# renegade-fi/mpc-jellyfish

Hardware: AMD Instinct MI355X
Metric: msm_g1_scalar_pairs_per_s (higher is better)
Workload: dtype u32 (381-bit Fq as 14 x 29-bit limbs, Montgomery)

## Files before the change

### mpc-jellyfish_amd/csrc/ecz.cuh

```cuda
#pragma once
#include "ecx.cuh"
#include "fz.cuh"

namespace mzk {

template <class Z>
struct AffineZ {
    Fz<Z> x, y;
    MZK_HD bool is_inf() const {
        int32_t a = 0;
#pragma unroll
        for (int i = 0; i < Z::ZN; i++) a |= x.l[i] | y.l[i];
        return a == 0;
    }
};

template <class Z>
struct XYZZZ {
    Fz<Z> x, y, zz, zzz;
    MZK_HD bool is_inf() const { return fz_is_zero(zz); }
    MZK_HD static XYZZZ inf() {
        XYZZZ r;
        r.x = Fz<Z>::one(); r.y = Fz<Z>::one(); r.zz = Fz<Z>::zero(); r.zzz = Fz<Z>::zero();
        return r;
    }
    MZK_HD static XYZZZ from_affine(const AffineZ<Z>& p) {
        if (p.is_inf()) return inf();
        XYZZZ r;
        r.x = p.x; r.y = p.y; r.zz = Fz<Z>::one(); r.zzz = Fz<Z>::one();
        return r;
    }
};

template <class Z>
MZK_HD void ecz_xy3(Fz<Z>& x3, Fz<Z>& y3, const Fz<Z>& a, const Fz<Z>& b_plus_2c, const Fz<Z>& q, const Fz<Z>& r, const Fz<Z>& y, const Fz<Z>& ppp) {
    x3 = fz_norm_wide(fz_sub(a, b_plus_2c));
    const Fz<Z> d = fz_norm(fz_sub(q, x3));
    y3 = fz_mul2(r, d, y, fz_neg(ppp));
}

template <class Z>
MZK_HD XYZZZ<Z> xyzzz_dbl_affine(const AffineZ<Z>& p) {
    XYZZZ<Z> r;
    const Fz<Z> u = fz_norm(fz_add(p.y, p.y));
    const Fz<Z> v = fz_sqr(u);
    const Fz<Z> w = fz_mul(u, v);
    const Fz<Z> s = fz_mul(p.x, v);
    const Fz<Z> x2 = fz_sqr(p.x);
    const Fz<Z> m = fz_norm_wide(fz_add(fz_add(x2, x2), x2));
    const Fz<Z> mm = fz_sqr(m);
    ecz_xy3<Z>(r.x, r.y, mm, fz_add(s, s), s, m, p.y, w);
    r.zz = v;
    r.zzz = w;
    return r;
}

template <class Z>
MZK_HD XYZZZ<Z> xyzzz_dbl(const XYZZZ<Z>& p) {
    if (p.is_inf()) return p;
    XYZZZ<Z> r;
    const Fz<Z> u = fz_norm(fz_add(p.y, p.y));
    const Fz<Z> v = fz_sqr(u);
    const Fz<Z> w = fz_mul(u, v);
    const Fz<Z> s = fz_mul(p.x, v);
    const Fz<Z> x2 = fz_sqr(p.x);
    const Fz<Z> m = fz_norm_wide(fz_add(fz_add(x2, x2), x2));
    const Fz<Z> mm = fz_sqr(m);
    ecz_xy3<Z>(r.x, r.y, mm, fz_add(s, s), s, m, p.y, w);
    r.zz = fz_mul(v, p.zz);
    r.zzz = fz_mul(w, p.zzz);
    return r;
}

template <class Z>
MZK_HD XYZZZ<Z> xyzzz_madd(const XYZZZ<Z>& p, const AffineZ<Z>& q, bool negate) {
    if (q.is_inf()) return p;
    const Fz<Z> qy = negate ? fz_neg(q.y) : q.y;
    if (p.is_inf()) {
        XYZZZ<Z> r;
        r.x = q.x; r.y = qy; r.zz = Fz<Z>::one(); r.zzz = Fz<Z>::one();
        return r;
    }
    const Fz<Z> u2 = fz_mul(q.x, p.zz);
    const Fz<Z> s2 = fz_mul(qy, p.zzz);
    const Fz<Z> pp_ = fz_norm(fz_sub(u2, p.x));
    const Fz<Z> rr_ = fz_norm(fz_sub(s2, p.y));
    const Fz<Z> pp = fz_sqr(pp_);
    const Fz<Z> rr2 = fz_sqr(rr_);
    if (fz_is_zero(pp)) {
        if (fz_is_zero(rr2)) {
            AffineZ<Z> qq;
            qq.x = q.x;
            qq.y = qy;
            return xyzzz_dbl_affine(qq);
        }
        return XYZZZ<Z>::inf();
    }
    XYZZZ<Z> r;
    const Fz<Z> ppp = fz_mul(pp_, pp);
    const Fz<Z> qv = fz_mul(p.x, pp);
    ecz_xy3<Z>(r.x, r.y, rr2, fz_add(ppp, fz_add(qv, qv)), qv, rr_, p.y, ppp);
    r.zz = fz_mul(p.zz, pp);
    r.zzz = fz_mul(p.zzz, ppp);
    return r;
}

template <class Z>
MZK_HD XYZZZ<Z> xyzzz_add(const XYZZZ<Z>& p, const XYZZZ<Z>& q) {
    if (q.is_inf()) return p;
    if (p.is_inf()) return q;
    const Fz<Z> u1 = fz_mul(p.x, q.zz), u2 = fz_mul(q.x, p.zz);
    const Fz<Z> s1 = fz_mul(p.y, q.zzz), s2 = fz_mul(q.y, p.zzz);
    const Fz<Z> pp_ = fz_norm(fz_sub(u2, u1));
    const Fz<Z> rr_ = fz_norm(fz_sub(s2, s1));
    const Fz<Z> pp = fz_sqr(pp_);
    const Fz<Z> rr2 = fz_sqr(rr_);
    if (fz_is_zero(pp)) {
        if (fz_is_zero(rr2)) return xyzzz_dbl(p);
        return XYZZZ<Z>::inf();
    }
    XYZZZ<Z> r;
    const Fz<Z> ppp = fz_mul(pp_, pp);
    const Fz<Z> qv = fz_mul(u1, pp);
    ecz_xy3<Z>(r.x, r.y, rr2, fz_add(ppp, fz_add(qv, qv)), qv, rr_, s1, ppp);
    r.zz = fz_mul(fz_mul(p.zz, q.zz), pp);
    r.zzz = fz_mul(fz_mul(p.zzz, q.zzz), ppp);
    return r;
}

#if defined(__HIPCC__)
template <int CTRL, class Z>
__device__ __forceinline__ Fz<Z> fz_quad_perm(const Fz<Z>& a) {
    Fz<Z> r;
#pragma unroll
    for (int i = 0; i < Z::ZN; i++) {
        r.l[i] = __builtin_amdgcn_update_dpp(0, a.l[i], CTRL, 0xF, 0xF, true);
        asm("" : "+v"(r.l[i]));
    }
    return r;
}
template <class Z>
__device__ __forceinline__ Fz<Z> fz_sel(bool c, const Fz<Z>& a, const Fz<Z>& b) {
    Fz<Z> r;
#pragma unroll
    for (int i = 0; i < Z::ZN; i++) r.l[i] = c ? a.l[i] : b.l[i];
    return r;
}

template <class Z>
__device__ __forceinline__ Fz<Z> xyzzz_add_quad(const Fz<Z>& ca, const Fz<Z>& cb, int role) {
    const bool r0 = role == 0, r1 = role == 1, hi = role >= 2;
    int special = (role == 2 && (fz_is_zero(ca) || fz_is_zero(cb))) ? 1 : 0;
    const Fz<Z> p1 = fz_mul(ca, fz_quad_perm<QP_SWAP2>(cb));
    const Fz<Z> d = fz_norm(fz_sub(fz_quad_perm<QP_SWAP2>(p1), p1));
    const Fz<Z> p2 = fz_mul(fz_sel(hi, ca, d), fz_sel(hi, cb, d));
    if (r0 && fz_is_zero(p2)) special = 1;
    special |= __builtin_amdgcn_update_dpp(0, special, QP_SWAP1, 0xF, 0xF, true);
    special |= __builtin_amdgcn_update_dpp(0, special, QP_SWAP2, 0xF, 0xF, true);
    if (special) {
        XYZZZ<Z> a, b;
        a.x = fz_quad_perm<QP_L0>(ca); a.y = fz_quad_perm<QP_L1>(ca); a.zz = fz_quad_perm<QP_L2>(ca); a.zzz = fz_quad_perm<QP_L3>(ca);
        b.x = fz_quad_perm<QP_L0>(cb); b.y = fz_quad_perm<QP_L1>(cb); b.zz = fz_quad_perm<QP_L2>(cb); b.zzz = fz_quad_perm<QP_L3>(cb);
        const XYZZZ<Z> r = xyzzz_add(a, b);
        return fz_sel(hi, fz_sel(role == 2, r.zz, r.zzz), fz_sel(r0, r.x, r.y));
    }
    const Fz<Z> pp = fz_quad_perm<QP_L0>(p2);
    const Fz<Z> u1 = fz_quad_perm<QP_L0>(p1);
    const Fz<Z> p3 = fz_mul(fz_sel(r0, d, fz_sel(r1, u1, p2)), pp);
    const Fz<Z> ppp = fz_quad_perm<QP_L0>(p3);
    const Fz<Z> x3 = fz_norm_wide(fz_sub(p2, fz_add(ppp, fz_add(p3, p3))));
    const Fz<Z> qx = fz_norm(fz_sub(p3, x3));
    const Fz<Z> s1 = fz_quad_perm<QP_L1>(p1);
    const Fz<Z> p4 = fz_mul(fz_sel(r0, s1, fz_sel(r1, d, p2)), fz_sel(r1, qx, ppp));
    const Fz<Z> y3 = fz_norm(fz_sub(p4, fz_quad_perm<QP_L0>(p4)));
    const Fz<Z> x3_0 = fz_quad_perm<QP_L1>(x3);
    return fz_sel(hi, fz_sel(role == 2, p3, p4), fz_sel(r0, x3_0, y3));
}
#endif

// ... 11 lines not shown
```

### mpc-jellyfish_amd/csrc/fz.cuh

```cuda
#pragma once
#include "fp.cuh"

namespace mzk {

template <class Z>
struct Fz {
    static constexpr int N = Z::ZN;
    int32_t l[N];
    MZK_HD static Fz zero() {
        Fz r;
#pragma unroll
        for (int i = 0; i < N; i++) r.l[i] = 0;
        return r;
    }
    MZK_HD static Fz from_const(const int32_t (&c)[Z::ZN]) {
        Fz r;
#pragma unroll
        for (int i = 0; i < N; i++) r.l[i] = c[i];
        return r;
    }
    MZK_HD static Fz one() { return from_const(Z::ZONE); }
};

MZK_HD int32_t fz_sext(uint32_t v) { return (int32_t)(v << 2) >> 2; }
template <class Z>
MZK_HD int32_t fz_p_limb(int i) {
    int32_t v = Z::ZP[i];
#if defined(__HIP_DEVICE_COMPILE__)
    asm("" : "+s"(v));
#endif
    return v;
}

template <class Z>
MZK_HD Fz<Z> fz_mul(const Fz<Z>& x, const Fz<Z>& y) {
    constexpr int N = Z::ZN;
    int32_t m[N], pl[N];
#pragma unroll
    for (int i = 0; i < N; i++) pl[i] = fz_p_limb<Z>(i);
    Fz<Z> t;
    int64_t acc = 0;
#pragma unroll
    for (int k = 0; k < N; k++) {
#pragma unroll
        for (int i = 0; i <= k; i++) acc += (int64_t)x.l[i] * y.l[k - i];
#pragma unroll
        for (int i = 0; i < k; i++) acc += (int64_t)m[i] * pl[k - i];
        m[k] = fz_sext((uint32_t)acc * Z::ZINV);
        acc += (int64_t)m[k] * pl[0];
        acc >>= Z::ZL;
    }
#pragma unroll
    for (int k = N; k < 2 * N - 1; k++) {
#pragma unroll
        for (int i = k - N + 1; i < N; i++) {
            acc += (int64_t)x.l[i] * y.l[k - i];
            acc += (int64_t)m[i] * pl[k - i];
        }
        t.l[k - N] = fz_sext((uint32_t)acc);
        acc = (acc + (1 << (Z::ZL - 1))) >> Z::ZL;
    }
    t.l[N - 1] = (int32_t)acc;
    return t;
}
template <class Z>
MZK_HD Fz<Z> fz_mul2(const Fz<Z>& x, const Fz<Z>& y, const Fz<Z>& u, const Fz<Z>& v) {
    constexpr int N = Z::ZN;
    int32_t m[N], pl[N];
#pragma unroll
    for (int i = 0; i < N; i++) pl[i] = fz_p_limb<Z>(i);
    Fz<Z> t;
    int64_t acc = 0;
#pragma unroll
    for (int k = 0; k < N; k++) {
#pragma unroll
        for (int i = 0; i <= k; i++) {
            acc += (int64_t)x.l[i] * y.l[k - i];
            acc += (int64_t)u.l[i] * v.l[k - i];
        }
#pragma unroll
        for (int i = 0; i < k; i++) acc += (int64_t)m[i] * pl[k - i];
        m[k] = fz_sext((uint32_t)acc * Z::ZINV);
        acc += (int64_t)m[k] * pl[0];
        acc >>= Z::ZL;
    }
#pragma unroll
    for (int k = N; k < 2 * N - 1; k++) {
#pragma unroll
        for (int i = k - N + 1; i < N; i++) {
            acc += (int64_t)x.l[i] * y.l[k - i];
            acc += (int64_t)u.l[i] * v.l[k - i];
            acc += (int64_t)m[i] * pl[k - i];
        }
        t.l[k - N] = fz_sext((uint32_t)acc);
        acc = (acc + (1 << (Z::ZL - 1))) >> Z::ZL;
    }
    t.l[N - 1] = (int32_t)acc;
    return t;
}
template <class Z>
MZK_HD Fz<Z> fz_sqr(const Fz<Z>& x) {
    constexpr int N = Z::ZN;
    int32_t m[N], pl[N], x2[N];
#pragma unroll
    for (int i = 0; i < N; i++) { pl[i] = fz_p_limb<Z>(i); x2[i] = x.l[i] * 2; }
    Fz<Z> t;
    int64_t acc = 0;
#pragma unroll
    for (int k = 0; k < N; k++) {
#pragma unroll
        for (int i = 0; 2 * i < k; i++) acc += (int64_t)x.l[i] * x2[k - i];
        if (k % 2 == 0) acc += (int64_t)x.l[k / 2] * x.l[k / 2];
#pragma unroll
        for (int i = 0; i < k; i++) acc += (int64_t)m[i] * pl[k - i];
        m[k] = fz_sext((uint32_t)acc * Z::ZINV);
        acc += (int64_t)m[k] * pl[0];
        acc >>= Z::ZL;
    }
#pragma unroll
    for (int k = N; k < 2 * N - 1; k++) {
#pragma unroll
        for (int i = k - N + 1; 2 * i < k; i++) acc += (int64_t)x.l[i] * x2[k - i];
        if (k % 2 == 0) acc += (int64_t)x.l[k / 2] * x.l[k / 2];
#pragma unroll
        for (int i = k - N + 1; i < N; i++) acc += (int64_t)m[i] * pl[k - i];
        t.l[k - N] = fz_sext((uint32_t)acc);
        acc = (acc + (1 << (Z::ZL - 1))) >> Z::ZL;
    }
    t.l[N - 1] = (int32_t)acc;
    return t;
}

template <class Z>
MZK_HD Fz<Z> fz_add(const Fz<Z>& a, const Fz<Z>& b) {
    Fz<Z> r;
#pragma unroll
    for (int i = 0; i < Z::ZN; i++) r.l[i] = a.l[i] + b.l[i];
    return r;
}
template <class Z>
MZK_HD Fz<Z> fz_sub(const Fz<Z>& a, const Fz<Z>& b) {
    Fz<Z> r;
#pragma unroll
    for (int i = 0; i < Z::ZN; i++) r.l[i] = a.l[i] - b.l[i];
    return r;
}
template <class Z>
MZK_HD Fz<Z> fz_neg(const Fz<Z>& a) {
    Fz<Z> r;
#pragma unroll
    for (int i = 0; i < Z::ZN; i++) r.l[i] = -a.l[i];
    return r;
}

template <class Z>
MZK_HD Fz<Z> fz_norm(const Fz<Z>& a) {
    constexpr int N = Z::ZN, L = Z::ZL;
    Fz<Z> r;
    r.l[0] = fz_sext((uint32_t)a.l[0]);
#pragma unroll
    for (int i = 1; i < N - 1; i++) r.l[i] = fz_sext((uint32_t)a.l[i]) + ((a.l[i - 1] + (1 << (L - 1))) >> L);
    r.l[N - 1] = a.l[N - 1] + ((a.l[N - 2] + (1 << (L - 1))) >> L);
    return r;
}
template <class Z>
MZK_HD Fz<Z> fz_norm_wide(const Fz<Z>& a) {
    constexpr int N = Z::ZN, L = Z::ZL;
    Fz<Z> r;
    r.l[0] = fz_sext((uint32_t)a.l[0]);
#pragma unroll
    for (int i = 1; i < N - 1; i++) r.l[i] = fz_sext((uint32_t)a.l[i]) + (((a.l[i - 1] >> (L - 1)) + 1) >> 1);
    r.l[N - 1] = a.l[N - 1] + (((a.l[N - 2] >> (L - 1)) + 1) >> 1);
    return r;
}
template <class Z>
MZK_HD Fz<Z> fz_carry(const Fz<Z>& a) {
    constexpr int N = Z::ZN, L = Z::ZL;
    Fz<Z> r;
    int32_t c = 0;
#pragma unroll
    for (int i = 0; i < N - 1; i++) {
        const int32_t t = a.l[i] + c;
        r.l[i] = fz_sext((uint32_t)t);
        c = ((t >> (L - 1)) + 1) >> 1;
    }
    r.l[N - 1] = a.l[N - 1] + c;
    return r;
}
template <class Z>
MZK_HD bool fz_is_zero(const Fz<Z>& a) {
    int32_t z = 0;
#pragma unroll
    for (int i = 0; i < Z::ZN; i++) z |= a.l[i];
    return z == 0;
}
template <class Z>
MZK_HD Fz<Z> fz_canonical(const Fz<Z>& a) {
    constexpr int N = Z::ZN, L = Z::ZL;
    constexpr int32_t MASK = (1 << L) - 1;
    Fz<Z> r;
    int32_t c = 0;
#pragma unroll
    for (int i = 0; i < N - 1; i++) {
        const int32_t t = a.l[i] + c;
        r.l[i] = t & MASK;
        c = t >> L;
    }
    r.l[N - 1] = a.l[N - 1] + c;
// ... 79 lines not shown
```

### mpc-jellyfish_amd/csrc/msm.cuh

```cuda
#pragma once
#include <hip/hip_runtime.h>

#include "ec.cuh"
#include "ecx.cuh"
#include "ecz.cuh"

namespace mzk {

constexpr int MSM_THREADS = 256;
constexpr int MSM_ACC_THREADS = 128;
constexpr uint32_t MSM_HEAVY_PER_THREAD = 16;
constexpr uint32_t MSM_HEAVY_RUN = MSM_ACC_THREADS * MSM_HEAVY_PER_THREAD;
constexpr uint32_t MSM_HEAVY_FANIN = MSM_ACC_THREADS * 32;
constexpr int MSM_HEAVY_COUNTERS = 6;
__host__ __device__ inline bool msm_is_heavy(uint32_t count, uint32_t cap) { return count > cap + MSM_HEAVY_RUN; }

inline int msm_choose_window(unsigned long long n) {
    int lg = 0;
    while ((1ull << (lg + 1)) <= n) lg++;
    int c = lg - 2;
    if (c < 4) c = 4;
    if (c > 16) c = 16;
    return c;
}
// ... 152 lines not shown
        order[(size_t)row * M + pos] = w * M + b;
    }
}

struct LongDesc;
struct HeavyRun;
__device__ __forceinline__ void msm_long_register(uint32_t w, uint32_t b, uint32_t c, uint32_t offs_t, int n_win, uint32_t cap, uint32_t desc_cap,
                                                  LongDesc* __restrict__ desc, uint32_t* __restrict__ desc_count, uint32_t run_cap,
                                                  uint32_t h1_cap, HeavyRun* __restrict__ heavy_runs);
__global__ __launch_bounds__(1024) void msm_order_place_kernel(const uint32_t* __restrict__ hist, const uint32_t* __restrict__ offs, uint32_t M,
                                                               const uint32_t* __restrict__ keycnt, uint32_t* __restrict__ keycur, uint32_t* __restrict__ order,
                                                               int n_win, uint32_t cap, uint32_t desc_cap, LongDesc* __restrict__ desc,
                                                               uint32_t* __restrict__ desc_count, uint32_t run_cap, uint32_t h1_cap, HeavyRun* __restrict__ heavy_runs,
                                                               bool global) {
    __shared__ uint32_t cnt[1024];
    __shared__ uint32_t part[1024];
    const uint32_t w = blockIdx.y, t = threadIdx.x;
    const uint32_t row = global ? 0u : w;
    const uint32_t lo = blockIdx.x * MSM_ORDER_SLICE, hi = min(M, lo + MSM_ORDER_SLICE);
    uint32_t total = 0;
    if (global) for (uint32_t s = 0; s < gridDim.y; s++) total += keycnt[(size_t)s * 1024 + t];
    else total = keycnt[(size_t)w * 1024 + t];
    part[t] = total;
    cnt[t] = 0;
    __syncthreads();
    for (int d = 1; d < 1024; d <<= 1) {
        uint32_t v = t >= (uint32_t)d ? part[t - d] : 0;
        __syncthreads();
        part[t] += v;
        __syncthreads();
    }
    const uint32_t key_start = part[t] - total;
    for (uint32_t b = lo + t; b < hi; b += 1024) atomicAdd(&cnt[order_key(hist[(size_t)w * M + b])], 1u);
    __syncthreads();
    const uint32_t mine = cnt[t];
    __syncthreads();
    cnt[t] = mine ? key_start + atomicAdd(&keycur[(size_t)row * 1024 + t], mine) : 0u;
    __syncthreads();
    for (uint32_t b = lo + t; b < hi; b += 1024) {
        const uint32_t c = hist[(size_t)w * M + b];
        const uint32_t pos = atomicAdd(&cnt[order_key(c)], 1u);
        order[(size_t)row * M + pos] = w * M + b;
        if (desc_count && c > cap) msm_long_register(w, b, c, offs[(size_t)w * M + b], n_win, cap, desc_cap, desc, desc_count, run_cap, h1_cap, heavy_runs);
    }
}

template <class FQ>
__device__ __forceinline__ Affine<Fp<FQ>> load_affine(const uint32_t* __restrict__ bases, unsigned long long idx) {
    Affine<Fp<FQ>> p;
    const uint32_t* src = bases + idx * (2 * FQ::N);
    p.x = load_fp<FQ>(src);
    p.y = load_fp<FQ>(src + FQ::N);
    return p;
}
template <class FQ>
__device__ __forceinline__ XYZZ<Fp<FQ>> load_xyzz(const uint32_t* __restrict__ buf, unsigned long long idx) {
    XYZZ<Fp<FQ>> p;
    const uint32_t* src = buf + idx * (4 * FQ::N);
    p.x = load_fp<FQ>(src);
    p.y = load_fp<FQ>(src + FQ::N);
    p.zz = load_fp<FQ>(src + 2 * FQ::N);
    p.zzz = load_fp<FQ>(src + 3 * FQ::N);
    return p;
}
template <class FQ>
__device__ __forceinline__ void store_xyzz(uint32_t* __restrict__ buf, unsigned long long idx, const XYZZ<Fp<FQ>>& p) {
    uint32_t* dst = buf + idx * (4 * FQ::N);
    store_fp<FQ>(dst, p.x);
    store_fp<FQ>(dst + FQ::N, p.y);
    store_fp<FQ>(dst + 2 * FQ::N, p.zz);
    store_fp<FQ>(dst + 3 * FQ::N, p.zzz);
}

template <class FQ>
struct EcFp {
    using Field = FQ;
    using Aff = Affine<Fp<FQ>>;
    using Pt = XYZZ<Fp<FQ>>;
    static constexpr int AFF_WORDS = 2 * FQ::N, PT_WORDS = 4 * FQ::N;
    static __device__ __forceinline__ Aff load_aff(const uint32_t* __restrict__ bases, unsigned long long idx) { return load_affine<FQ>(bases, idx); }
    static __device__ __forceinline__ Pt load_pt(const uint32_t* __restrict__ buf, unsigned long long idx) { return load_xyzz<FQ>(buf, idx); }
    static __device__ __forceinline__ void store_pt(uint32_t* __restrict__ buf, unsigned long long idx, const Pt& p) { store_xyzz<FQ>(buf, idx, p); }
    static __device__ __forceinline__ Pt inf() { return Pt::inf(); }
    static __device__ __forceinline__ Pt madd(const Pt& a, Aff q, bool negate) {
        if (negate) q.y = neg(q.y);
        return xyzz_madd(a, q);
    }
    static __device__ __forceinline__ Pt add(const Pt& a, const Pt& b) { return xyzz_add(a, b); }
    static __device__ __forceinline__ XYZZ<Fp<FQ>> to_boundary(const Pt& p) { return p; }
};

template <class X>
__device__ __forceinline__ void load_words(uint32_t* dst, const uint32_t* __restrict__ src, int n_words) {
    for (int i = 0; i < n_words / 4; i++) {
        const uint4 v = reinterpret_cast<const uint4*>(src)[i];
        dst[4 * i] = v.x; dst[4 * i + 1] = v.y; dst[4 * i + 2] = v.z; dst[4 * i + 3] = v.w;
    }
}

template <class X>
struct EcFx {
    using Field = X;
    using Aff = AffineX<X>;
    using Pt = XYZZX<X>;
    using Fe = Fx<X>;
    static constexpr int LIMBS = X::XN, SLOT_WORDS = X::XN;
    static constexpr int AFF_WORDS = 2 * X::XN, PT_WORDS = 4 * X::XN;
    static_assert((4 * X::XN) % 4 == 0 && (2 * X::XN) % 2 == 0, "points are whole 16-byte / 8-byte words");
    static __device__ __forceinline__ Aff load_aff(const uint32_t* __restrict__ bases, unsigned long long idx) {
        uint32_t w[AFF_WORDS];
        if constexpr (AFF_WORDS % 4 == 0) {
            const uint4* src = reinterpret_cast<const uint4*>(bases + idx * AFF_WORDS);
#pragma unroll
            for (int i = 0; i < AFF_WORDS / 4; i++) {
                const uint4 v = src[i];
                w[4 * i] = v.x; w[4 * i + 1] = v.y; w[4 * i + 2] = v.z; w[4 * i + 3] = v.w;
            }
        } else {
            const uint2* src = reinterpret_cast<const uint2*>(bases + idx * AFF_WORDS);
#pragma unroll
            for (int i = 0; i < AFF_WORDS / 2; i++) {
                const uint2 v = src[i];
                w[2 * i] = v.x; w[2 * i + 1] = v.y;
            }
        }
        Aff p;
#pragma unroll
        for (int i = 0; i < X::XN; i++) { p.x.l[i] = w[i]; p.y.l[i] = w[X::XN + i]; }
        return p;
    }
    static __device__ __forceinline__ Pt load_pt(const uint32_t* __restrict__ buf, unsigned long long idx) {
        uint32_t w[PT_WORDS];
        const uint4* src = reinterpret_cast<const uint4*>(buf + idx * PT_WORDS);
#pragma unroll
        for (int i = 0; i < PT_WORDS / 4; i++) {
            const uint4 v = src[i];
            w[4 * i] = v.x; w[4 * i + 1] = v.y; w[4 * i + 2] = v.z; w[4 * i + 3] = v.w;
        }
        Pt p;
#pragma unroll
        for (int i = 0; i < X::XN; i++) {
            p.x.l[i] = w[i]; p.y.l[i] = w[X::XN + i]; p.zz.l[i] = w[2 * X::XN + i]; p.zzz.l[i] = w[3 * X::XN + i];
        }
        return p;
    }
    static __device__ __forceinline__ void store_pt(uint32_t* __restrict__ buf, unsigned long long idx, const Pt& p) {
        uint32_t w[PT_WORDS];
#pragma unroll
        for (int i = 0; i < X::XN; i++) {
            w[i] = p.x.l[i]; w[X::XN + i] = p.y.l[i]; w[2 * X::XN + i] = p.zz.l[i]; w[3 * X::XN + i] = p.zzz.l[i];
        }
        uint4* dst = reinterpret_cast<uint4*>(buf + idx * PT_WORDS);
#pragma unroll
        for (int i = 0; i < PT_WORDS / 4; i++) dst[i] = make_uint4(w[4 * i], w[4 * i + 1], w[4 * i + 2], w[4 * i + 3]);
    }
    static __device__ __forceinline__ Pt inf() { return Pt::inf(); }
    static __device__ __forceinline__ Pt madd(const Pt& a, const Aff& q, bool negate) { return xyzzx_madd(a, q, negate); }
    static __device__ __forceinline__ Pt add(const Pt& a, const Pt& b) { return xyzzx_add(a, b); }
    static __device__ __forceinline__ XYZZ<Fp<X>> to_boundary(const Pt& p) { return xyzzx_to_boundary(p); }
    static __device__ __forceinline__ Fe add_quad(const Fe& ca, const Fe& cb, int role) { return xyzzx_add_quad<X>(ca, cb, role); }
};

template <class Z>
struct EcFz {
    using Field = Z;
    using Aff = AffineZ<Z>;
    using Pt = XYZZZ<Z>;
    using Fe = Fz<Z>;
    static constexpr int LIMBS = Z::ZN, SLOT_WORDS = Z::ZN + 1;
    static constexpr int AFF_WORDS = 2 * SLOT_WORDS, PT_WORDS = 4 * SLOT_WORDS;
    static_assert(AFF_WORDS % 4 == 0, "points are whole 16-byte words");
    static __device__ __forceinline__ Aff load_aff(const uint32_t* __restrict__ bases, unsigned long long idx) {
        uint32_t w[AFF_WORDS];
        const uint4* src = reinterpret_cast<const uint4*>(bases + idx * AFF_WORDS);
#pragma unroll
        for (int i = 0; i < AFF_WORDS / 4; i++) {
            const uint4 v = src[i];
            w[4 * i] = v.x; w[4 * i + 1] = v.y; w[4 * i + 2] = v.z; w[4 * i + 3] = v.w;
        }
        Aff p;
#pragma unroll
        for (int i = 0; i < LIMBS; i++) { p.x.l[i] = (int32_t)w[i]; p.y.l[i] = (int32_t)w[SLOT_WORDS + i]; }
        return p;
    }
    static __device__ __forceinline__ void store_aff(uint32_t* __restrict__ bases, unsigned long long idx, const Aff& p) {
        uint32_t w[AFF_WORDS];
#pragma unroll
        for (int i = 0; i < LIMBS; i++) { w[i] = (uint32_t)p.x.l[i]; w[SLOT_WORDS + i] = (uint32_t)p.y.l[i]; }
        w[LIMBS] = 0; w[SLOT_WORDS + LIMBS] = 0;
        uint4* dst = reinterpret_cast<uint4*>(bases + idx * AFF_WORDS);
#pragma unroll
        for (int i = 0; i < AFF_WORDS / 4; i++) dst[i] = make_uint4(w[4 * i], w[4 * i + 1], w[4 * i + 2], w[4 * i + 3]);
    }
    static __device__ __forceinline__ Pt load_pt(const uint32_t* __restrict__ buf, unsigned long long idx) {
        uint32_t w[PT_WORDS];
        const uint4* src = reinterpret_cast<const uint4*>(buf + idx * PT_WORDS);
#pragma unroll
        for (int i = 0; i < PT_WORDS / 4; i++) {
            const uint4 v = src[i];
            w[4 * i] = v.x; w[4 * i + 1] = v.y; w[4 * i + 2] = v.z; w[4 * i + 3] = v.w;
        }
        Pt p;
#pragma unroll
        for (int i = 0; i < LIMBS; i++) {
            p.x.l[i] = (int32_t)w[i]; p.y.l[i] = (int32_t)w[SLOT_WORDS + i];
            p.zz.l[i] = (int32_t)w[2 * SLOT_WORDS + i]; p.zzz.l[i] = (int32_t)w[3 * SLOT_WORDS + i];
        }
        return p;
    }
    static __device__ __forceinline__ void store_pt(uint32_t* __restrict__ buf, unsigned long long idx, const Pt& p) {
        uint32_t w[PT_WORDS];
#pragma unroll
        for (int i = 0; i < LIMBS; i++) {
            w[i] = (uint32_t)p.x.l[i]; w[SLOT_WORDS + i] = (uint32_t)p.y.l[i];
            w[2 * SLOT_WORDS + i] = (uint32_t)p.zz.l[i]; w[3 * SLOT_WORDS + i] = (uint32_t)p.zzz.l[i];
        }
#pragma unroll
        for (int k = 0; k < 4; k++) w[k * SLOT_WORDS + LIMBS] = 0;
        uint4* dst = reinterpret_cast<uint4*>(buf + idx * PT_WORDS);
#pragma unroll
        for (int i = 0; i < PT_WORDS / 4; i++) dst[i] = make_uint4(w[4 * i], w[4 * i + 1], w[4 * i + 2], w[4 * i + 3]);
    }
    static __device__ __forceinline__ Pt inf() { return Pt::inf(); }
    static __device__ __forceinline__ Pt madd(const Pt& a, const Aff& q, bool negate) { return xyzzz_madd(a, q, negate); }
    static __device__ __forceinline__ Pt add(const Pt& a, const Pt& b) { return xyzzz_add(a, b); }
    static __device__ __forceinline__ XYZZ<Fp<Z>> to_boundary(const Pt& p) { return xyzzz_to_boundary(p); }
    static __device__ __forceinline__ Fe add_quad(const Fe& ca, const Fe& cb, int role) { return xyzzz_add_quad<Z>(ca, cb, role); }
};

template <class Z>
__global__ __launch_bounds__(MSM_THREADS) void srs_to_internal_z_kernel(const uint32_t* __restrict__ xy, unsigned long long n, uint32_t* __restrict__ out) {
    const unsigned long long i = (unsigned long long)blockIdx.x * MSM_THREADS + threadIdx.x;
    if (i >= n) return;
    const Fp<Z> x = load_fp<Z>(xy + i * 2 * Z::N), y = load_fp<Z>(xy + i * 2 * Z::N + Z::N);
    AffineZ<Z> p;
    p.x = fz_from_boundary<Z>(x);
    p.y = fz_from_boundary<Z>(y);
    EcFz<Z>::store_aff(out, i, p);
}

template <class X>
__global__ __launch_bounds__(MSM_THREADS) void srs_to_internal_kernel(const uint32_t* __restrict__ xy, unsigned long long n, uint32_t* __restrict__ out) {
    const unsigned long long i = (unsigned long long)blockIdx.x * MSM_THREADS + threadIdx.x;
    if (i >= n) return;
    const Fp<X> x = load_fp<X>(xy + i * 2 * X::N), y = load_fp<X>(xy + i * 2 * X::N + X::N);
    const Fx<X> fx = fx_from_boundary<X>(x), fy = fx_from_boundary<X>(y);
    uint32_t* dst = out + i * 2 * X::XN;
#pragma unroll
    for (int k = 0; k < X::XN; k++) { dst[k] = fx.l[k]; dst[X::XN + k] = fy.l[k]; }
}

template <class EC>
__global__ __launch_bounds__(MSM_ACC_THREADS) void msm_accumulate_kernel(const uint32_t* __restrict__ bases, unsigned long long n,
                                                                          const uint32_t* __restrict__ offs, const uint32_t* __restrict__ hist,
                                                                          const uint32_t* __restrict__ sorted, const uint32_t* __restrict__ order,
                                                                          uint32_t M, int n_win, uint32_t cap, uint32_t* __restrict__ long_count,
                                                                          uint32_t* __restrict__ buckets, uint8_t* __restrict__ occ) {
    if (long_count && blockIdx.x == 0)
        for (unsigned i = threadIdx.x; i < (unsigned)n_win * (1 + MSM_HEAVY_COUNTERS); i += MSM_ACC_THREADS) long_count[i] = 0u;
    const unsigned long long t0 = (unsigned long long)blockIdx.x * MSM_ACC_THREADS + threadIdx.x;
    if (t0 >= (unsigned long long)n_win * M) return;
    const uint32_t tb = order[t0];
    const unsigned long long t = tb, w = tb / M;
    const uint32_t start = offs[t];
    const uint32_t h = hist[t];
    const uint32_t cnt = msm_is_heavy(h, cap) ? 0u : min(h, cap);
    const uint32_t* list = sorted + w * n + start;
    typename EC::Pt acc = EC::inf();
    for (uint32_t k = 0; k < cnt; k++) {
        const uint32_t e = list[k];
        acc = EC::madd(acc, EC::load_aff(bases, e & 0x7fffffffu), (e >> 31) != 0);
    }
    const bool empty = acc.is_inf();
    occ[t] = empty ? 0 : 1;
    if (!empty) EC::store_pt(buckets, t, acc);
}

template <class EC, bool ONE_SET>
__global__ __launch_bounds__(MSM_ACC_THREADS) void msm_accumulate_split_kernel(const uint32_t* __restrict__ bases, unsigned long long n,
                                                                                const uint32_t* __restrict__ offs, const uint32_t* __restrict__ hist,
                                                                                const uint32_t* __restrict__ sorted, const uint32_t* __restrict__ order,
                                                                                uint32_t M, int n_win, uint32_t cap, int log_split, uint32_t* __restrict__ long_count,
                                                                                uint32_t* __restrict__ sub, unsigned long long rank0,
                                                                                uint32_t* __restrict__ buckets, uint8_t* __restrict__ occ) {
    if (long_count && blockIdx.x == 0)
        for (unsigned i = threadIdx.x; i < (unsigned)n_win * (1 + MSM_HEAVY_COUNTERS); i += MSM_ACC_THREADS) long_count[i] = 0u;
    const unsigned long long t1 = (unsigned long long)blockIdx.x * MSM_ACC_THREADS + threadIdx.x;
    const bool whole = t1 < rank0;
    const unsigned long long u = whole ? 0ull : t1 - rank0;
    const unsigned long long t0 = whole ? t1 : rank0 + (u >> log_split);
    if (t0 >= (unsigned long long)n_win * M) return;
    const uint32_t S = whole ? 1u : 1u << log_split, part = whole ? 0u : (uint32_t)(u & (S - 1));
    const uint32_t tb = order[t0];
    const unsigned long long t = tb, w = ONE_SET ? 0ull : tb / M;
    const uint32_t start = offs[t];
    const uint32_t h = hist[t];
    const uint32_t cnt = msm_is_heavy(h, cap) ? 0u : min(h, cap);
    const uint32_t* list = sorted + w * n + start;
    typename EC::Pt acc = EC::inf();
    for (uint32_t k = part; k < cnt; k += S) {
        const uint32_t e = list[k];
        acc = EC::madd(acc, EC::load_aff(bases, e & 0x7fffffffu), (e >> 31) != 0);
    }
    if (whole) {
        const bool empty = acc.is_inf();
        occ[t] = empty ? 0 : 1;
        if (!empty) EC::store_pt(buckets, t, acc);
    } else {
        EC::store_pt(sub, u, acc);
    }
}
template <class EC>
__device__ __forceinline__ void pt_lds_put(uint32_t* lds, int slot, const typename EC::Pt& p) {
    constexpr int N = EC::LIMBS;
#pragma unroll
    for (int i = 0; i < N; i++) {
        lds[i * MSM_ACC_THREADS + slot] = p.x.l[i];
        lds[(N + i) * MSM_ACC_THREADS + slot] = p.y.l[i];
        lds[(2 * N + i) * MSM_ACC_THREADS + slot] = p.zz.l[i];
        lds[(3 * N + i) * MSM_ACC_THREADS + slot] = p.zzz.l[i];
    }
}
template <class EC>
__device__ __forceinline__ typename EC::Pt pt_lds_get(const uint32_t* lds, int slot) {
    constexpr int N = EC::LIMBS;
    typename EC::Pt p;
#pragma unroll
    for (int i = 0; i < N; i++) {
        p.x.l[i] = lds[i * MSM_ACC_THREADS + slot];
        p.y.l[i] = lds[(N + i) * MSM_ACC_THREADS + slot];
        p.zz.l[i] = lds[(2 * N + i) * MSM_ACC_THREADS + slot];
        p.zzz.l[i] = lds[(3 * N + i) * MSM_ACC_THREADS + slot];
    }
    return p;
}
template <class EC, bool ONE_SET>
__global__ __launch_bounds__(MSM_ACC_THREADS) void msm_split_combine_kernel(const uint32_t* __restrict__ sub, unsigned long long n_buckets, int log_split,
                                                                             const uint32_t* __restrict__ order, unsigned long long rank0,
                                                                             uint32_t* __restrict__ buckets, uint8_t* __restrict__ occ) {
    __shared__ uint32_t lds[MSM_ACC_THREADS * EC::PT_WORDS];
    const int tid = threadIdx.x;
    const unsigned long long total = n_buckets << log_split;
    const unsigned long long base = (unsigned long long)blockIdx.x * (2 * MSM_ACC_THREADS);
    typename EC::Pt acc = EC::inf();
#pragma unroll 1
    for (int lvl = 0; lvl < log_split; lvl++) {
        const bool mine = tid < (MSM_ACC_THREADS >> lvl) && base + ((unsigned long long)(2 * tid) << lvl) < total;
        typename EC::Pt a = EC::inf(), b = EC::inf();
        if (lvl == 0) {
            if (mine) { a = EC::load_pt(sub, base + 2ull * tid); b = EC::load_pt(sub, base + 2ull * tid + 1); }
        } else {
            __syncthreads();
            if (mine) { a = pt_lds_get<EC>(lds, 2 * tid); b = pt_lds_get<EC>(lds, 2 * tid + 1); }
            __syncthreads();
        }
        if (mine) {
            acc = EC::add(a, b);
            if (lvl == log_split - 1) {
                const unsigned long long t = order[rank0 + (base >> log_split) + tid];
                const bool empty = acc.is_inf();
                occ[t] = empty ? 0 : 1;
                if (!empty) EC::store_pt(buckets, t, acc);
            } else pt_lds_put<EC>(lds, tid, acc);
        }
    }
}

struct LongDesc { uint32_t bucket, start, len, idx_in_run, run_len; };

struct HeavyRun { uint32_t src, n, dest, p1; };
constexpr uint32_t MSM_HEAVY_DEST_PART = 0x80000000u;
constexpr int MSM_HEAVY_JOBS = 8;
struct HeavyJob {
    const uint32_t* bases;
    const uint32_t* sorted;
    unsigned long long n;
    const HeavyRun* runs;
    const uint32_t* count;
    uint32_t *h1, *h2, *h3, *buckets;
    uint8_t* occ;
    uint32_t run_cap, h1_cap, M;
    const LongDesc* desc;
    const uint32_t* desc_count;
    uint32_t* parts;
    uint32_t desc_cap;
};
struct HeavyJobs { HeavyJob j[MSM_HEAVY_JOBS]; };
__device__ __forceinline__ void msm_heavy_push(uint32_t b, uint32_t start, uint32_t rem, uint32_t run_cap, uint32_t h1_cap, uint32_t* __restrict__ cnt,
                                               HeavyRun* __restrict__ runs0, HeavyRun* __restrict__ runsB, HeavyRun* __restrict__ runsC) {
    const uint32_t n1 = (rem + MSM_HEAVY_RUN - 1) / MSM_HEAVY_RUN;
    const uint32_t need = (rem + MSM_HEAVY_PER_THREAD - 1) / MSM_HEAVY_PER_THREAD + n1;
    const uint32_t p1 = atomicAdd(&cnt[5], need);
    if (p1 + need > h1_cap) return;
    const uint32_t r0 = atomicAdd(&cnt[0], n1);
    if (r0 + n1 > run_cap) return;
    constexpr uint32_t PER_RUN = MSM_HEAVY_RUN / MSM_HEAVY_PER_THREAD;
    const uint32_t p2 = atomicAdd(&cnt[3], n1);
    for (uint32_t i = 0; i < n1; i++)
        runs0[r0 + i] = HeavyRun{start + i * MSM_HEAVY_RUN, min(MSM_HEAVY_RUN, rem - i * MSM_HEAVY_RUN), MSM_HEAVY_DEST_PART | (p2 + i), p1 + i * PER_RUN};
    const uint32_t n2 = (n1 + MSM_HEAVY_FANIN - 1) / MSM_HEAVY_FANIN;
    const uint32_t rb = atomicAdd(&cnt[1], n2);
    if (n2 == 1) { runsB[rb] = HeavyRun{p2, n1, b, 0}; return; }
    const uint32_t p3 = atomicAdd(&cnt[4], n2);
    for (uint32_t j = 0; j < n2; j++)
        runsB[rb + j] = HeavyRun{p2 + j * MSM_HEAVY_FANIN, min(MSM_HEAVY_FANIN, n1 - j * MSM_HEAVY_FANIN), MSM_HEAVY_DEST_PART | (p3 + j), 0};
    runsC[atomicAdd(&cnt[2], 1u)] = HeavyRun{p3, n2, b, 0};
}

__device__ __forceinline__ void msm_long_register(uint32_t w, uint32_t b, uint32_t c, uint32_t offs_t, int n_win, uint32_t cap, uint32_t desc_cap,
                                                  LongDesc* __restrict__ desc, uint32_t* __restrict__ desc_count, uint32_t run_cap,
                                                  uint32_t h1_cap, HeavyRun* __restrict__ heavy_runs);

__global__ __launch_bounds__(256) void msm_long_find_kernel(const uint32_t* __restrict__ hist, const uint32_t* __restrict__ offs, uint32_t M, int n_win,
                                                            uint32_t cap, uint32_t desc_cap, LongDesc* __restrict__ desc,
                                                            uint32_t* __restrict__ desc_count, uint32_t run_cap, uint32_t h1_cap, HeavyRun* __restrict__ heavy_runs) {
    const unsigned long long t = (unsigned long long)blockIdx.x * 256 + threadIdx.x;
    if (t >= (unsigned long long)n_win * M) return;
    const uint32_t c = hist[t];
    if (c <= cap) return;
    msm_long_register((uint32_t)(t / M), (uint32_t)(t % M), c, offs[t], n_win, cap, desc_cap, desc, desc_count, run_cap, h1_cap, heavy_runs);
}
__device__ __forceinline__ void msm_long_register(uint32_t w, uint32_t b, uint32_t c, uint32_t offs_t, int n_win, uint32_t cap, uint32_t desc_cap,
                                                  LongDesc* __restrict__ desc, uint32_t* __restrict__ desc_count, uint32_t run_cap,
                                                  uint32_t h1_cap, HeavyRun* __restrict__ heavy_runs) {
    if (msm_is_heavy(c, cap)) {
        HeavyRun* base = heavy_runs + (size_t)w * 3 * run_cap;
        msm_heavy_push(b, offs_t, c, run_cap, h1_cap, desc_count + n_win + (size_t)w * MSM_HEAVY_COUNTERS, base, base + run_cap, base + 2 * (size_t)run_cap);
        return;
    }
    const uint32_t nch = (c - cap + cap - 1) / cap;
    const uint32_t pos = atomicAdd(&desc_count[w], nch);
    if (pos + nch > desc_cap) {
        for (uint32_t i = pos; i < desc_cap; i++) desc[(size_t)w * desc_cap + i] = LongDesc{b, offs_t, 0u, 1u, 0u};
        return;
    }
    for (uint32_t j = 0; j < nch; j++) {
        LongDesc d;
        d.bucket = b;
        d.start = offs_t + cap * (j + 1);
        d.len = min(cap, c - cap * (j + 1));
        d.idx_in_run = j;
        d.run_len = nch;
        desc[(size_t)w * desc_cap + pos + j] = d;
    }
}

template <class EC>
__global__ __launch_bounds__(MSM_ACC_THREADS) void msm_long_chunk_kernel(const uint32_t* __restrict__ bases, unsigned long long n,
                                                                          const uint32_t* __restrict__ sorted, const LongDesc* __restrict__ desc,
                                                                          const uint32_t* __restrict__ desc_count, uint32_t desc_cap,
                                                                          uint32_t* __restrict__ parts) {
    const uint32_t w = blockIdx.y;
    const uint32_t i = blockIdx.x * MSM_ACC_THREADS + threadIdx.x;
    if (i >= min(desc_count[w], desc_cap)) return;
    const LongDesc d = desc[(size_t)w * desc_cap + i];
    const uint32_t* list = sorted + (size_t)w * n + d.start;
    typename EC::Pt acc = EC::inf();
    for (uint32_t k = 0; k < d.len; k++) {
        const uint32_t e = list[k];
        acc = EC::madd(acc, EC::load_aff(bases, e & 0x7fffffffu), (e >> 31) != 0);
    }
    EC::store_pt(parts, (size_t)w * desc_cap + i, acc);
}

template <class EC>
__global__ __launch_bounds__(MSM_ACC_THREADS) void msm_rare_leaf_kernel(HeavyJobs jobs, uint32_t long_blocks) {
    const HeavyJob& jb = jobs.j[blockIdx.z];
    const uint32_t w = blockIdx.y, t = threadIdx.x;
    const bool is_long = blockIdx.x < long_blocks;
    const uint32_t heavy_cnt = is_long ? 0u : min(jb.count[(size_t)w * MSM_HEAVY_COUNTERS], jb.run_cap);
    const HeavyRun* runs = jb.runs + (size_t)w * 3 * jb.run_cap;
    const uint32_t r_step = is_long ? 1u : gridDim.x - long_blocks;
    uint32_t r = is_long ? 0u : blockIdx.x - long_blocks;
    for (;; r += r_step) {
        const uint32_t* list;
        uint32_t cnt;
        uint32_t* out;
        size_t out_idx;
        if (is_long) {
            if (r) break;
            const uint32_t i = blockIdx.x * MSM_ACC_THREADS + t;
            if (i >= min(jb.desc_count[w], jb.desc_cap)) break;
            const LongDesc d = jb.desc[(size_t)w * jb.desc_cap + i];
            list = jb.sorted + (size_t)w * jb.n + d.start;
            cnt = d.len;
            out = jb.parts;
            out_idx = (size_t)w * jb.desc_cap + i;
        } else {
            if (r >= heavy_cnt) break;
            const HeavyRun run = runs[r];
            const uint32_t lo = t * MSM_HEAVY_PER_THREAD;
            if (lo >= run.n) continue;
            list = jb.sorted + (size_t)w * jb.n + run.src + lo;
            cnt = min(run.n, lo + MSM_HEAVY_PER_THREAD) - lo;
            out = jb.h1;
            out_idx = (size_t)w * jb.h1_cap + run.p1 + t;
        }
        typename EC::Pt acc = EC::inf();
        for (uint32_t k = 0; k < cnt; k++) {
            const uint32_t e = list[k];
            acc = EC::madd(acc, EC::load_aff(jb.bases, e & 0x7fffffffu), (e >> 31) != 0);
        }
        EC::store_pt(out, out_idx, acc);
    }
}

template <class EC>
__global__ __launch_bounds__(MSM_ACC_THREADS) void msm_long_combine_kernel(HeavyJobs jobs) {
    const HeavyJob& jb = jobs.j[blockIdx.z];
    const LongDesc* __restrict__ desc = jb.desc;
    const uint32_t* __restrict__ desc_count = jb.desc_count;
    const uint32_t desc_cap = jb.desc_cap, M = jb.M;
    const uint32_t* __restrict__ parts = jb.parts;
    uint32_t* __restrict__ buckets = jb.buckets;
    uint8_t* __restrict__ occ = jb.occ;
    const uint32_t w = blockIdx.y;
    const uint32_t cnt = min(desc_count[w], desc_cap);
    const LongDesc* dw = desc + (size_t)w * desc_cap;
    const size_t pbase = (size_t)w * desc_cap;
    for (uint32_t i = blockIdx.x * MSM_ACC_THREADS + threadIdx.x; i < cnt; i += gridDim.x * MSM_ACC_THREADS) {
        const LongDesc d = dw[i];
        if (d.idx_in_run != 0) continue;
        const size_t bi = (size_t)w * M + d.bucket;
        typename EC::Pt acc = occ[bi] ? EC::load_pt(buckets, bi) : EC::inf();
        for (uint32_t j = 0; j < d.run_len; j++) acc = EC::add(acc, EC::load_pt(parts, pbase + i + j));
        const bool empty = acc.is_inf();
        occ[bi] = empty ? 0 : 1;
        if (!empty) EC::store_pt(buckets, bi, acc);
    }
}

template <class EC>
__global__ __launch_bounds__(MSM_ACC_THREADS) void msm_heavy_chunk_kernel(HeavyJobs jobs) {
    const HeavyJob& jb = jobs.j[blockIdx.z];
    const uint32_t w = blockIdx.y, t = threadIdx.x, run_cap = jb.run_cap;
    const uint32_t cnt = min(jb.count[(size_t)w * MSM_HEAVY_COUNTERS], run_cap);
    const HeavyRun* runs = jb.runs + (size_t)w * 3 * run_cap;
    for (uint32_t r = blockIdx.x; r < cnt; r += gridDim.x) {
        const HeavyRun run = runs[r];
        const uint32_t lo = t * MSM_HEAVY_PER_THREAD;
        if (lo >= run.n) continue;
        const uint32_t hi = min(run.n, lo + MSM_HEAVY_PER_THREAD);
        const uint32_t* list = jb.sorted + (size_t)w * jb.n + run.src;
        typename EC::Pt acc = EC::inf();
        for (uint32_t k = lo; k < hi; k++) {
            const uint32_t e = list[k];
            acc = EC::madd(acc, EC::load_aff(jb.bases, e & 0x7fffffffu), (e >> 31) != 0);
        }
        EC::store_pt(jb.h1, (size_t)w * jb.h1_cap + run.p1 + t, acc);
    }
}
template <class EC>
__global__ __launch_bounds__(MSM_ACC_THREADS) void msm_heavy_reduce_kernel(HeavyJobs jobs, int level ) {
    __shared__ uint32_t lds[MSM_ACC_THREADS * EC::PT_WORDS];
    const HeavyJob& jb = jobs.j[blockIdx.z];
    const uint32_t w = blockIdx.y, run_cap = jb.run_cap, M = jb.M;
    const int tid = threadIdx.x;
    const uint32_t* parts_in = level == 0 ? jb.h1 : (level == 1 ? jb.h2 : jb.h3);
    uint32_t* parts_out = level == 0 ? jb.h2 : jb.h3;
    uint32_t* buckets = jb.buckets;
    uint8_t* occ = jb.occ;
    const uint32_t cnt = min(jb.count[(size_t)w * MSM_HEAVY_COUNTERS + level], run_cap);
    const HeavyRun* runs = jb.runs + ((size_t)w * 3 + level) * run_cap;
    const size_t in_base = (size_t)w * (level == 0 ? jb.h1_cap : run_cap), out_base = (size_t)w * run_cap;
    for (uint32_t r = blockIdx.x; r < cnt; r += gridDim.x) {
        const HeavyRun run = runs[r];
        const uint32_t n_items = level == 0 ? (run.n + MSM_HEAVY_PER_THREAD - 1) / MSM_HEAVY_PER_THREAD : run.n;
        const size_t src = in_base + (level == 0 ? (size_t)run.p1 : (size_t)run.src);
        const int per = (int)((n_items + MSM_ACC_THREADS - 1) / MSM_ACC_THREADS);
        int log_w = 0;
        while ((1u << log_w) < n_items && log_w < 7) log_w++;
        typename EC::Pt acc = (uint32_t)tid < n_items ? EC::load_pt(parts_in, src + tid) : EC::inf();
        const bool to_bucket = !(run.dest & MSM_HEAVY_DEST_PART);
        const size_t bi = (size_t)w * M + run.dest;
        const int n_steps = (per - 1) + log_w;
#pragma unroll 1
        for (int s = 0; s < n_steps; s++) {
            typename EC::Pt a = EC::inf(), b = EC::inf();
            bool act = false;
            if (s < per - 1) {
                const uint32_t q = (uint32_t)tid + (uint32_t)(s + 1) * MSM_ACC_THREADS;
                if (q < n_items) { a = acc; b = EC::load_pt(parts_in, src + q); act = true; }
            } else {
                const int l = s - (per - 1);
                __syncthreads();
                if (tid < ((1 << log_w) >> l)) pt_lds_put<EC>(lds, tid, acc);
                __syncthreads();
                if (tid < ((1 << log_w) >> (l + 1))) { a = pt_lds_get<EC>(lds, 2 * tid); b = pt_lds_get<EC>(lds, 2 * tid + 1); act = true; }
            }
            if (act) acc = EC::add(a, b);
        }
        if (tid == 0) {
            if (to_bucket) {
                const bool empty = acc.is_inf();
                occ[bi] = empty ? 0 : 1;
                if (!empty) EC::store_pt(buckets, bi, acc);
            } else {
                EC::store_pt(parts_out, out_base + (run.dest & ~MSM_HEAVY_DEST_PART), acc);
            }
        }
    }
}

template <class EC>
__device__ __forceinline__ void fold_one(uint32_t* __restrict__ buckets, uint8_t* __restrict__ occ, unsigned long long ia, unsigned long long ib) {
    if (!occ[ib]) return;
    typename EC::Pt b = EC::load_pt(buckets, ib);
    if (!occ[ia]) {
        EC::store_pt(buckets, ia, b);
        occ[ia] = 1;
        return;
    }
    typename EC::Pt a = EC::load_pt(buckets, ia);
    EC::store_pt(buckets, ia, EC::add(a, b));
}
template <class EC>
__global__ __launch_bounds__(MSM_ACC_THREADS) void msm_fold_kernel(uint32_t* __restrict__ buckets, uint8_t* __restrict__ occ, uint32_t M, uint32_t h, int nseg, int n_win) {
    const unsigned long long t = (unsigned long long)blockIdx.x * MSM_ACC_THREADS + threadIdx.x;
    const unsigned long long per_win = (unsigned long long)nseg * h;
    if (t >= per_win * n_win) return;
    const unsigned long long w = t / per_win, r = t % per_win;
    const uint32_t seg = (uint32_t)(r / h), i = (uint32_t)(r % h);
    const unsigned long long base = w * M + (seg ? (M >> seg) : 0u);
    fold_one<EC>(buckets, occ, base + i, base + h + i);
}

template <class EC>
__global__ __launch_bounds__(MSM_ACC_THREADS) void msm_fold2_kernel(uint32_t* __restrict__ buckets, uint8_t* __restrict__ occ, uint32_t M, uint32_t h, int nseg, int n_win) {
    const uint32_t q = h >> 1;
    const unsigned long long t = (unsigned long long)blockIdx.x * MSM_ACC_THREADS + threadIdx.x;
    const unsigned long long per_win = (unsigned long long)nseg * q;
// ... 361 lines not shown
```

Baseline: 348.1 million.

## Peel first bucket point out of madd loop and move madd edge cases off hot path

Bucket accumulation loops now initialise the accumulator from the first affine point instead of adding it to infinity, through a shared msm_sum_run helper. xyzzz_madd computes the generic path first and merges its infinity and doubling checks into one branch that calls a separate rare-case function, to cut divergence and code size in the hot loop. The Montgomery multiply inner products now go through an fz_mac helper wrapped in __builtin_annotation, meant to steer how the compiler schedules the 64-bit accumulations. The annotation builtin may not behave as intended on the AMD backend, and the generic madd path now runs even when an input is at infinity.

```diff
diff --git a/mpc-jellyfish_amd/csrc/ecz.cuh b/mpc-jellyfish_amd/csrc/ecz.cuh
--- a/mpc-jellyfish_amd/csrc/ecz.cuh
+++ b/mpc-jellyfish_amd/csrc/ecz.cuh
@@ -73,28 +73,36 @@
 }
 
 template <class Z>
+MZK_HD XYZZZ<Z> xyzzz_from_affine_signed(const AffineZ<Z>& q, bool negate) {
+    AffineZ<Z> s;
+    s.x = q.x;
+    s.y = negate ? fz_neg(q.y) : q.y;
+    return XYZZZ<Z>::from_affine(s);
+}
+
+template <class Z>
+MZK_HD XYZZZ<Z> xyzzz_madd_rare(const XYZZZ<Z>& p, const AffineZ<Z>& qs, const Fz<Z>& pp, const Fz<Z>& rr2) {
+    if (qs.is_inf()) return p;
+    if (p.is_inf()) return XYZZZ<Z>::from_affine(qs);
+    if (fz_is_zero(rr2)) return xyzzz_dbl_affine(qs);
+    (void)pp;
+    return XYZZZ<Z>::inf();
+}
+
+template <class Z>
 MZK_HD XYZZZ<Z> xyzzz_madd(const XYZZZ<Z>& p, const AffineZ<Z>& q, bool negate) {
-    if (q.is_inf()) return p;
     const Fz<Z> qy = negate ? fz_neg(q.y) : q.y;
-    if (p.is_inf()) {
-        XYZZZ<Z> r;
-        r.x = q.x; r.y = qy; r.zz = Fz<Z>::one(); r.zzz = Fz<Z>::one();
-        return r;
-    }
     const Fz<Z> u2 = fz_mul(q.x, p.zz);
     const Fz<Z> s2 = fz_mul(qy, p.zzz);
     const Fz<Z> pp_ = fz_norm(fz_sub(u2, p.x));
     const Fz<Z> rr_ = fz_norm(fz_sub(s2, p.y));
     const Fz<Z> pp = fz_sqr(pp_);
     const Fz<Z> rr2 = fz_sqr(rr_);
-    if (fz_is_zero(pp)) {
-        if (fz_is_zero(rr2)) {
-            AffineZ<Z> qq;
-            qq.x = q.x;
-            qq.y = qy;
-            return xyzzz_dbl_affine(qq);
-        }
-        return XYZZZ<Z>::inf();
+    if (q.is_inf() | p.is_inf() | fz_is_zero(pp)) {
+        AffineZ<Z> qs;
+        qs.x = q.x;
+        qs.y = qy;
+        return xyzzz_madd_rare(p, qs, pp, rr2);
     }
     XYZZZ<Z> r;
     const Fz<Z> ppp = fz_mul(pp_, pp);
diff --git a/mpc-jellyfish_amd/csrc/fz.cuh b/mpc-jellyfish_amd/csrc/fz.cuh
--- a/mpc-jellyfish_amd/csrc/fz.cuh
+++ b/mpc-jellyfish_amd/csrc/fz.cuh
@@ -32,6 +32,13 @@
     return v;
 }
 
+#if defined(__HIP_DEVICE_COMPILE__)
+__device__ __forceinline__ int64_t fz_keep(int64_t v) { return __builtin_annotation(v, "fz"); }
+#else
+inline int64_t fz_keep(int64_t v) { return v; }
+#endif
+MZK_HD int64_t fz_mac(int64_t acc, int32_t a, int32_t b) { return fz_keep(acc + (int64_t)a * b); }
+
 template <class Z>
 MZK_HD Fz<Z> fz_mul(const Fz<Z>& x, const Fz<Z>& y) {
     constexpr int N = Z::ZN;
@@ -43,19 +50,19 @@
 #pragma unroll
     for (int k = 0; k < N; k++) {
 #pragma unroll
-        for (int i = 0; i <= k; i++) acc += (int64_t)x.l[i] * y.l[k - i];
-#pragma unroll
-        for (int i = 0; i < k; i++) acc += (int64_t)m[i] * pl[k - i];
+        for (int i = 0; i <= k; i++) acc = fz_mac(acc, x.l[i], y.l[k - i]);
+#pragma unroll
+        for (int i = 0; i < k; i++) acc = fz_mac(acc, m[i], pl[k - i]);
         m[k] = fz_sext((uint32_t)acc * Z::ZINV);
-        acc += (int64_t)m[k] * pl[0];
+        acc = fz_mac(acc, m[k], pl[0]);
         acc >>= Z::ZL;
     }
 #pragma unroll
     for (int k = N; k < 2 * N - 1; k++) {
 #pragma unroll
         for (int i = k - N + 1; i < N; i++) {
-            acc += (int64_t)x.l[i] * y.l[k - i];
-            acc += (int64_t)m[i] * pl[k - i];
+            acc = fz_mac(acc, x.l[i], y.l[k - i]);
+            acc = fz_mac(acc, m[i], pl[k - i]);
         }
         t.l[k - N] = fz_sext((uint32_t)acc);
         acc = (acc + (1 << (Z::ZL - 1))) >> Z::ZL;
@@ -75,22 +82,22 @@
     for (int k = 0; k < N; k++) {
 #pragma unroll
         for (int i = 0; i <= k; i++) {
-            acc += (int64_t)x.l[i] * y.l[k - i];
-            acc += (int64_t)u.l[i] * v.l[k - i];
+            acc = fz_mac(acc, x.l[i], y.l[k - i]);
+            acc = fz_mac(acc, u.l[i], v.l[k - i]);
         }
 #pragma unroll
-        for (int i = 0; i < k; i++) acc += (int64_t)m[i] * pl[k - i];
+        for (int i = 0; i < k; i++) acc = fz_mac(acc, m[i], pl[k - i]);
         m[k] = fz_sext((uint32_t)acc * Z::ZINV);
-        acc += (int64_t)m[k] * pl[0];
+        acc = fz_mac(acc, m[k], pl[0]);
         acc >>= Z::ZL;
     }
 #pragma unroll
     for (int k = N; k < 2 * N - 1; k++) {
 #pragma unroll
         for (int i = k - N + 1; i < N; i++) {
-            acc += (int64_t)x.l[i] * y.l[k - i];
-            acc += (int64_t)u.l[i] * v.l[k - i];
-            acc += (int64_t)m[i] * pl[k - i];
+            acc = fz_mac(acc, x.l[i], y.l[k - i]);
+            acc = fz_mac(acc, u.l[i], v.l[k - i]);
+            acc = fz_mac(acc, m[i], pl[k - i]);
         }
         t.l[k - N] = fz_sext((uint32_t)acc);
         acc = (acc + (1 << (Z::ZL - 1))) >> Z::ZL;
@@ -109,21 +116,21 @@
 #pragma unroll
     for (int k = 0; k < N; k++) {
 #pragma unroll
-        for (int i = 0; 2 * i < k; i++) acc += (int64_t)x.l[i] * x2[k - i];
-        if (k % 2 == 0) acc += (int64_t)x.l[k / 2] * x.l[k / 2];
-#pragma unroll
-        for (int i = 0; i < k; i++) acc += (int64_t)m[i] * pl[k - i];
+        for (int i = 0; 2 * i < k; i++) acc = fz_mac(acc, x.l[i], x2[k - i]);
+        if (k % 2 == 0) acc = fz_mac(acc, x.l[k / 2], x.l[k / 2]);
+#pragma unroll
+        for (int i = 0; i < k; i++) acc = fz_mac(acc, m[i], pl[k - i]);
         m[k] = fz_sext((uint32_t)acc * Z::ZINV);
-        acc += (int64_t)m[k] * pl[0];
+        acc = fz_mac(acc, m[k], pl[0]);
         acc >>= Z::ZL;
     }
 #pragma unroll
     for (int k = N; k < 2 * N - 1; k++) {
 #pragma unroll
-        for (int i = k - N + 1; 2 * i < k; i++) acc += (int64_t)x.l[i] * x2[k - i];
-        if (k % 2 == 0) acc += (int64_t)x.l[k / 2] * x.l[k / 2];
-#pragma unroll
-        for (int i = k - N + 1; i < N; i++) acc += (int64_t)m[i] * pl[k - i];
+        for (int i = k - N + 1; 2 * i < k; i++) acc = fz_mac(acc, x.l[i], x2[k - i]);
+        if (k % 2 == 0) acc = fz_mac(acc, x.l[k / 2], x.l[k / 2]);
+#pragma unroll
+        for (int i = k - N + 1; i < N; i++) acc = fz_mac(acc, m[i], pl[k - i]);
         t.l[k - N] = fz_sext((uint32_t)acc);
         acc = (acc + (1 << (Z::ZL - 1))) >> Z::ZL;
     }
diff --git a/mpc-jellyfish_amd/csrc/msm.cuh b/mpc-jellyfish_amd/csrc/msm.cuh
--- a/mpc-jellyfish_amd/csrc/msm.cuh
+++ b/mpc-jellyfish_amd/csrc/msm.cuh
@@ -258,6 +258,7 @@
     static __device__ __forceinline__ Pt load_pt(const uint32_t* __restrict__ buf, unsigned long long idx) { return load_xyzz<FQ>(buf, idx); }
     static __device__ __forceinline__ void store_pt(uint32_t* __restrict__ buf, unsigned long long idx, const Pt& p) { store_xyzz<FQ>(buf, idx, p); }
     static __device__ __forceinline__ Pt inf() { return Pt::inf(); }
+    static constexpr bool FIRST_OUTSIDE = false;
     static __device__ __forceinline__ Pt madd(const Pt& a, Aff q, bool negate) {
         if (negate) q.y = neg(q.y);
         return xyzz_madd(a, q);
@@ -331,6 +332,7 @@
         for (int i = 0; i < PT_WORDS / 4; i++) dst[i] = make_uint4(w[4 * i], w[4 * i + 1], w[4 * i + 2], w[4 * i + 3]);
     }
     static __device__ __forceinline__ Pt inf() { return Pt::inf(); }
+    static constexpr bool FIRST_OUTSIDE = false;
     static __device__ __forceinline__ Pt madd(const Pt& a, const Aff& q, bool negate) { return xyzzx_madd(a, q, negate); }
     static __device__ __forceinline__ Pt add(const Pt& a, const Pt& b) { return xyzzx_add(a, b); }
     static __device__ __forceinline__ XYZZ<Fp<X>> to_boundary(const Pt& p) { return xyzzx_to_boundary(p); }
@@ -398,6 +400,8 @@
         for (int i = 0; i < PT_WORDS / 4; i++) dst[i] = make_uint4(w[4 * i], w[4 * i + 1], w[4 * i + 2], w[4 * i + 3]);
     }
     static __device__ __forceinline__ Pt inf() { return Pt::inf(); }
+    static constexpr bool FIRST_OUTSIDE = true;
+    static __device__ __forceinline__ Pt first(const Aff& q, bool negate) { return xyzzz_from_affine_signed(q, negate); }
     static __device__ __forceinline__ Pt madd(const Pt& a, const Aff& q, bool negate) { return xyzzz_madd(a, q, negate); }
     static __device__ __forceinline__ Pt add(const Pt& a, const Pt& b) { return xyzzz_add(a, b); }
     static __device__ __forceinline__ XYZZ<Fp<Z>> to_boundary(const Pt& p) { return xyzzz_to_boundary(p); }
@@ -424,6 +428,24 @@
     uint32_t* dst = out + i * 2 * X::XN;
 #pragma unroll
     for (int k = 0; k < X::XN; k++) { dst[k] = fx.l[k]; dst[X::XN + k] = fy.l[k]; }
+}
+
+template <class EC>
+__device__ __forceinline__ typename EC::Pt msm_sum_run(const uint32_t* __restrict__ bases, const uint32_t* __restrict__ list, uint32_t k, uint32_t cnt,
+                                                       uint32_t step) {
+    typename EC::Pt acc = EC::inf();
+    if constexpr (EC::FIRST_OUTSIDE) {
+        if (k < cnt) {
+            const uint32_t e = list[k];
+            acc = EC::first(EC::load_aff(bases, e & 0x7fffffffu), (e >> 31) != 0);
+            k += step;
+        }
+    }
+    for (; k < cnt; k += step) {
+        const uint32_t e = list[k];
+        acc = EC::madd(acc, EC::load_aff(bases, e & 0x7fffffffu), (e >> 31) != 0);
+    }
+    return acc;
 }
 
 template <class EC>
@@ -442,11 +464,7 @@
     const uint32_t h = hist[t];
     const uint32_t cnt = msm_is_heavy(h, cap) ? 0u : min(h, cap);
     const uint32_t* list = sorted + w * n + start;
-    typename EC::Pt acc = EC::inf();
-    for (uint32_t k = 0; k < cnt; k++) {
-        const uint32_t e = list[k];
-        acc = EC::madd(acc, EC::load_aff(bases, e & 0x7fffffffu), (e >> 31) != 0);
-    }
+    const typename EC::Pt acc = msm_sum_run<EC>(bases, list, 0, cnt, 1u);
     const bool empty = acc.is_inf();
     occ[t] = empty ? 0 : 1;
     if (!empty) EC::store_pt(buckets, t, acc);
@@ -473,11 +491,7 @@
     const uint32_t h = hist[t];
     const uint32_t cnt = msm_is_heavy(h, cap) ? 0u : min(h, cap);
     const uint32_t* list = sorted + w * n + start;
-    typename EC::Pt acc = EC::inf();
-    for (uint32_t k = part; k < cnt; k += S) {
-        const uint32_t e = list[k];
-        acc = EC::madd(acc, EC::load_aff(bases, e & 0x7fffffffu), (e >> 31) != 0);
-    }
+    const typename EC::Pt acc = msm_sum_run<EC>(bases, list, part, cnt, S);
     if (whole) {
         const bool empty = acc.is_inf();
         occ[t] = empty ? 0 : 1;
@@ -631,11 +645,7 @@
     if (i >= min(desc_count[w], desc_cap)) return;
     const LongDesc d = desc[(size_t)w * desc_cap + i];
     const uint32_t* list = sorted + (size_t)w * n + d.start;
-    typename EC::Pt acc = EC::inf();
-    for (uint32_t k = 0; k < d.len; k++) {
-        const uint32_t e = list[k];
-        acc = EC::madd(acc, EC::load_aff(bases, e & 0x7fffffffu), (e >> 31) != 0);
-    }
+    const typename EC::Pt acc = msm_sum_run<EC>(bases, list, 0, d.len, 1u);
     EC::store_pt(parts, (size_t)w * desc_cap + i, acc);
 }
 
@@ -672,11 +682,7 @@
             out = jb.h1;
             out_idx = (size_t)w * jb.h1_cap + run.p1 + t;
         }
-        typename EC::Pt acc = EC::inf();
-        for (uint32_t k = 0; k < cnt; k++) {
-            const uint32_t e = list[k];
-            acc = EC::madd(acc, EC::load_aff(jb.bases, e & 0x7fffffffu), (e >> 31) != 0);
-        }
+        const typename EC::Pt acc = msm_sum_run<EC>(jb.bases, list, 0, cnt, 1u);
         EC::store_pt(out, out_idx, acc);
     }
 }
@@ -718,11 +724,7 @@
         if (lo >= run.n) continue;
         const uint32_t hi = min(run.n, lo + MSM_HEAVY_PER_THREAD);
         const uint32_t* list = jb.sorted + (size_t)w * jb.n + run.src;
-        typename EC::Pt acc = EC::inf();
-        for (uint32_t k = lo; k < hi; k++) {
-            const uint32_t e = list[k];
-            acc = EC::madd(acc, EC::load_aff(jb.bases, e & 0x7fffffffu), (e >> 31) != 0);
-        }
+        const typename EC::Pt acc = msm_sum_run<EC>(jb.bases, list, lo, hi, 1u);
         EC::store_pt(jb.h1, (size_t)w * jb.h1_cap + run.p1 + t, acc);
     }
 }
```

New measurement: 349.9 million, median of 6. Within noise of the previous version (+0.5%).
